# fchchen/omni-recall-rag

Measured on AMD Instinct MI355X. Metric: queries/sec at top-k=10 over N x 3072-d chunks; score delta vs C# reference in `parity`, higher is better.
Workload: dtype i8 screen + f32*f32->f64 exact re-score; 1 GPU; C3: 10000000 chunks x 3072-d fp32 on one GPU, batch=256 queries per step, top-k=10, full hybrid (cosine+keyword+recency), candidate_limit=corpus; corpus_rows=10000000

## Files before the change

omni-recall-rag_amd/csrc/orr_api.hip:

```cpp
#include <hip/hip_runtime.h>

#include <algorithm>
#include <cmath>
#include <cstdarg>
#include <cstdio>
#include <chrono>
#include <pthread.h>
#include <dlfcn.h>
#include <atomic>
#include <condition_variable>
#include <functional>
#include <cstring>
#include <limits>
#include <mutex>
#include <shared_mutex>
#include <deque>
#include <new>
#include <numeric>
#include <string>
#include <string_view>
#include <thread>
#include <unordered_map>
#include <vector>

// ... 95 lines not shown

}

struct orr_index {
    int device = 0;
    int32_t dim = 0;
    int64_t row_base = 0;
    hipStream_t stream = nullptr;
    hipStream_t stream_kw = nullptr;
    hipStream_t stream_aux = nullptr;
    hipEvent_t ev_bm_clean = nullptr;
    bool bm_clean_pending = false;
    bool kw_counters_clean = false;
    const void *kw_counters_of[2] = {nullptr, nullptr};
    hipEvent_t ev_inputs = nullptr, ev_kw_done = nullptr, ev_main_ready = nullptr, ev_range[15] = {};
    std::mutex mu;

    int64_t n_rows = 0, cap_rows = 0;
    float *d_emb = nullptr;
    int64_t *d_created = nullptr;
    int64_t *d_row_ids = nullptr;
    uint64_t *d_cstart = nullptr;
    uint32_t *d_clen = nullptr;
    uint8_t *d_pool = nullptr;
    uint64_t pool_len = 0, pool_cap = 0;
    double *d_norm_b = nullptr;
    int64_t n_tokens = 0;
    uint8_t *d_vpool = nullptr;
    uint64_t *d_vstart = nullptr;
    uint32_t *d_vlen = nullptr;
// ... 22 lines not shown
    int opt_shard_pass = 0;
    int opt_shard_topk = 0;
    int sample_boost = 1;
    DevBuf emb_shadow;
    bool shadow_ready = false, shadow_failed = false;
    DevBuf emb_i8, i8_scale, i8_rel_err, i8_rel_hat, i8_rowf;
    bool i8_ready = false, i8_failed = false;
    std::vector<int64_t> dead;
    DevBuf d_dead;
    int64_t dead_before = 0;
    const orr_index *parent = nullptr;
    std::vector<std::pair<int64_t, int64_t>> id_index;

    DevBuf ws_q, ws_dot, ws_dotf, ws_sel, ws_cand, ws_qc, ws_rowc, ws_tau, ws_qsplit, ws_fcnt, ws_fbuf, ws_fqf, ws_fany, ws_tsL, ws_tskey, ws_qtiled, ws_fdot, ws_pbuf, ws_psel, ws_q8, ws_q8s1, ws_q8err, ws_zero, ws_norm_a;
    DevBuf ws_keys_a, ws_keys_b, ws_vals_a, ws_vals_b, ws_sort_tmp, ws_raw, ws_src_start, ws_qsub;
    DevBuf ws_vmatch, ws_bitmaps, ws_hits, ws_counter, ws_meta, ws_tickets, ws_kwalias;
    size_t bitmaps_clean = 0;
    const void *bitmaps_clean_of = nullptr;
    PinnedBuf pin_meta, pin_q, pin_qc, pin_cand, pin_norm, pin_cnt, pin_kwcnt;
    hipEvent_t ev_q = nullptr;

    LanePool lanes{this};
    bool internal_lane = false;
    std::atomic<int> user_views{0};

    int profiling = 0;
    std::vector<KernelStat> stats;
    std::vector<PendingEvent> pending;
    std::vector<hipEvent_t> event_pool;
};

// ... 342 lines not shown
    HIP_TRY(hipGetDeviceProperties(&prop, cfg->device));
    if (strncmp(prop.gcnArchName, "gfx950", 6) != 0)
        return fail(ORR_EDEVICE, "device %d is %s; this library carries gfx950 code only", cfg->device, prop.gcnArchName);
    orr_index *idx = new (std::nothrow) orr_index();
    if (!idx) return fail(ORR_ENOMEM, "out of host memory");
    idx->device = cfg->device;
    idx->dim = cfg->dim;
    idx->row_base = cfg->row_base;
    if (hipSetDevice(idx->device) != hipSuccess || hipStreamCreateWithFlags(&idx->stream, hipStreamNonBlocking) != hipSuccess ||
        hipStreamCreateWithFlags(&idx->stream_kw, hipStreamNonBlocking) != hipSuccess ||
        hipStreamCreateWithFlags(&idx->stream_aux, hipStreamNonBlocking) != hipSuccess ||
        hipEventCreateWithFlags(&idx->ev_bm_clean, hipEventDisableTiming) != hipSuccess ||
        hipEventCreateWithFlags(&idx->ev_inputs, hipEventDisableTiming) != hipSuccess ||
        hipEventCreateWithFlags(&idx->ev_kw_done, hipEventDisableTiming) != hipSuccess ||
        hipEventCreateWithFlags(&idx->ev_main_ready, hipEventDisableTiming) != hipSuccess ||
        !create_range_events(idx->ev_range) ||
        hipEventCreateWithFlags(&idx->ev_q, hipEventDisableTiming) != hipSuccess) {
        orr_index_destroy(idx);
        return fail(ORR_EDEVICE, "cannot create streams on device %d", cfg->device);
    }
    if (cfg->capacity_rows > 0) {
        int r = ensure_row_capacity(idx, cfg->capacity_rows);
        if (r != ORR_OK) { orr_index_destroy(idx); return r; }
    }
    *out = idx;
    return ORR_OK;
}

void orr_index_destroy(orr_index *idx)
{
// ... 5 lines not shown
            LanePool::Exclusive all(&idx->lanes);
            views = idx->lanes.drain();
            idx->lanes.set_max_lanes(1);
        }
        for (orr_index *l : views) orr_index_destroy(l);
    }
    (void)hipSetDevice(idx->device);
    if (idx->stream) (void)hipStreamSynchronize(idx->stream);
    if (idx->stream_kw) (void)hipStreamSynchronize(idx->stream_kw);
    if (idx->stream_aux) (void)hipStreamSynchronize(idx->stream_aux);
    if (idx->ev_bm_clean) (void)hipEventDestroy(idx->ev_bm_clean);
    if (idx->stream_aux) (void)hipStreamDestroy(idx->stream_aux);
    if (idx->ev_inputs) (void)hipEventDestroy(idx->ev_inputs);
    if (idx->ev_kw_done) (void)hipEventDestroy(idx->ev_kw_done);
    if (idx->ev_main_ready) (void)hipEventDestroy(idx->ev_main_ready);
    for (hipEvent_t e : idx->ev_range) if (e) (void)hipEventDestroy(e);
    if (idx->stream_kw) (void)hipStreamDestroy(idx->stream_kw);
    for (auto &pe : idx->pending) { (void)hipEventDestroy(pe.start); (void)hipEventDestroy(pe.stop); }
    for (auto e : idx->event_pool) (void)hipEventDestroy(e);
    if (!idx->is_view) {
        if (idx->d_emb) (void)hipFree(idx->d_emb);
        if (idx->d_created) (void)hipFree(idx->d_created);
        if (idx->d_row_ids) (void)hipFree(idx->d_row_ids);
        if (idx->d_cstart) (void)hipFree(idx->d_cstart);
        if (idx->d_clen) (void)hipFree(idx->d_clen);
        if (idx->d_pool) (void)hipFree(idx->d_pool);
        if (idx->d_norm_b) (void)hipFree(idx->d_norm_b);
        if (idx->d_vpool) (void)hipFree(idx->d_vpool);
        if (idx->d_vstart) (void)hipFree(idx->d_vstart);
        if (idx->d_vlen) (void)hipFree(idx->d_vlen);
// ... 866 lines not shown
    v->device = parent->device; v->dim = parent->dim; v->row_base = parent->row_base;
    v->n_rows = parent->n_rows; v->cap_rows = parent->cap_rows;
    v->d_emb = parent->d_emb; v->d_created = parent->d_created; v->d_row_ids = parent->d_row_ids; v->d_norm_b = parent->d_norm_b;
    v->n_tokens = parent->n_tokens; v->d_vpool = parent->d_vpool; v->d_vstart = parent->d_vstart; v->d_vlen = parent->d_vlen;
    v->d_post_off = parent->d_post_off; v->d_post_rows = parent->d_post_rows; v->n_postings = parent->n_postings;
    v->sealed = true;
    copy_options(parent, v);
    borrow_shadows(parent, v);
    if (hipStreamCreateWithFlags(&v->stream, hipStreamNonBlocking) != hipSuccess ||
        hipStreamCreateWithFlags(&v->stream_kw, hipStreamNonBlocking) != hipSuccess ||
        hipStreamCreateWithFlags(&v->stream_aux, hipStreamNonBlocking) != hipSuccess ||
        hipEventCreateWithFlags(&v->ev_bm_clean, hipEventDisableTiming) != hipSuccess ||
        hipEventCreateWithFlags(&v->ev_inputs, hipEventDisableTiming) != hipSuccess ||
        hipEventCreateWithFlags(&v->ev_kw_done, hipEventDisableTiming) != hipSuccess ||
        hipEventCreateWithFlags(&v->ev_main_ready, hipEventDisableTiming) != hipSuccess ||
        !create_range_events(v->ev_range) ||
        hipEventCreateWithFlags(&v->ev_q, hipEventDisableTiming) != hipSuccess) {
        v->internal_lane = true;
        orr_index_destroy(v);
        return fail(ORR_EDEVICE, "cannot create streams on device %d", parent->device);
    }
    v->internal_lane = internal;
    if (!internal) parent->user_views.fetch_add(1);
    *out = v;
    return ORR_OK;
}

int orr_index_screen_dots(orr_index *idx, int32_t B, int32_t dim, const float *q, float *out)
{
    if (!idx || !q || !out || B <= 0) return fail(ORR_EINVAL, "orr_index_screen_dots: bad argument");
// ... 185 lines not shown
    void done()
    {
        if (!on || ++calls % 64 != 0) return;
        fprintf(stderr, "[orr host ms/call] query_setup+cos_launch %.3f | keyword_prep+launch %.3f | norms+consts %.3f | select_launches %.3f | "
                        "wait_gpu %.3f | finish %.3f\n", acc[0] / 64, acc[1] / 64, acc[2] / 64, acc[3] / 64, acc[4] / 64, acc[5] / 64);
        for (double &x : acc) x = 0;
    }
};
thread_local HostTiming g_ht;

struct KwSide {
    orr::KwView view{nullptr, 0, nullptr, nullptr, nullptr};
    size_t bm_bytes = 0, bm_clean_before = 0;
    bool overflow_possible = false;
    uint32_t max_hits = 0;
};

int launch_keyword_side(orr_index *idx, const BatchArgs &a, const std::vector<uint32_t> &qoff, KwSide &out)
{
    const int32_t B = a.B;
    const uint32_t t_begin = qoff[0], n_terms_total = qoff[(size_t)B] - qoff[0];
    if (n_terms_total == 0) return ORR_OK;
    {

        std::vector<std::string_view> dterms;
        dterms.reserve(n_terms_total);
        uint32_t table_size = 16;
        while (table_size < 2 * n_terms_total + 2) table_size <<= 1;
        std::vector<uint32_t> table(table_size, 0xFFFFFFFFu);
        std::vector<uint32_t> qmeta((size_t)n_terms_total + (size_t)B + 1);
// ... 99 lines not shown
        size_t bm_clean = idx->bitmaps_clean_of == idx->ws_bitmaps.p ? idx->bitmaps_clean : 0;
        idx->bitmaps_clean = 0;
        idx->bitmaps_clean_of = idx->ws_bitmaps.p;
        out.bm_clean_before = bm_clean;
        ORR_TRY(idx->ws_hits.reserve(sizeof(orr::KwHit) * (size_t)max_hits));
        ORR_TRY(idx->ws_counter.reserve(sizeof(unsigned long long)));
        ORR_TRY(idx->pin_kwcnt.reserve(sizeof(unsigned long long)));
        *idx->pin_kwcnt.as<unsigned long long>() = 0ull;
        hipStream_t k = idx->stream_kw;
        uint8_t *dm = idx->ws_meta.as<uint8_t>();
        HIP_TRY(hipMemcpyAsync(dm, hm, meta_bytes, hipMemcpyHostToDevice, k));
        const bool counters_clean = idx->kw_counters_clean && idx->kw_counters_of[0] == idx->ws_counter.p;
        idx->kw_counters_clean = false;
        if (!counters_clean) HIP_TRY(hipMemsetAsync(idx->ws_counter.p, 0, sizeof(unsigned long long), k));
        bool bitmaps_settled = false;
        auto settle_bitmaps = [&]() -> int {
            if (bitmaps_settled) return ORR_OK;
            bitmaps_settled = true;
            if (idx->bm_clean_pending) {
                HIP_TRY(hipStreamWaitEvent(k, idx->ev_bm_clean, 0));
                idx->bm_clean_pending = false;
            }
            if (bm_clean < out.bm_bytes)
                HIP_TRY(hipMemsetAsync(static_cast<uint8_t *>(idx->ws_bitmaps.p) + bm_clean, 0, out.bm_bytes - bm_clean, k));
            return ORR_OK;
        };
        if (V > 0) {
            const orr::ScanTerm *d_terms = reinterpret_cast<const orr::ScanTerm *>(dm + off_terms);
            {
                Timed t(idx, "vocab_match", 0.0, k);
                if (vocab_lookup) {
                    const uint32_t *lk = reinterpret_cast<const uint32_t *>(dm + off_lk);
                    HIP_TRY(orr::launch_vocab_match_lookup(idx->d_vpool, idx->d_vstart, idx->d_vlen, V,
                                                           reinterpret_cast<const orr::MatchTerm *>(dm + off_match), lk, lk + 8, lk + 8 + TT,
                                                           reinterpret_cast<const uint32_t *>(dm + off_bloom), idx->d_post_off,
                                                           idx->ws_counter.as<unsigned long long>(), idx->ws_hits.as<orr::KwHit>(), max_hits, k));
                } else {
// ... 16 lines not shown
                {
                    Timed t(idx, "vocab_scan", 0.0, k);
                    HIP_TRY(orr::launch_vocab_scan(idx->d_vpool, idx->vlong_start.as<uint64_t>() + n_mid, idx->vlong_len.as<uint32_t>() + n_mid, VS,
                                                   dm + off_pool, d_terms, (int32_t)TT, reinterpret_cast<const uint32_t *>(dm + off_iota),
                                                   idx->ws_vmatch.as<uint16_t>(), k));
                }
                {
                    Timed t(idx, "vocab_hits", 0.0, k);
                    HIP_TRY(orr::launch_vocab_hits(idx->ws_vmatch.as<uint16_t>(), VS, (int32_t)TT, idx->vlong_id.as<uint32_t>() + n_mid, idx->d_post_off,
                                                   idx->ws_counter.as<unsigned long long>(), idx->ws_hits.as<orr::KwHit>(), max_hits, k));
                }
            }
            const uint8_t *skip = nullptr;
            if (idx->n_tok_bm > 0 && idx->tok_bm_words == words) {
                const size_t o_tok = sizeof(uint32_t) * (size_t)TT, o_off = (2 * o_tok + 7) / 8 * 8, o_alias = o_off + sizeof(int64_t) * (size_t)TT;
                ORR_TRY(idx->ws_kwalias.reserve(o_alias + (size_t)TT + 16));
                uint8_t *wa = idx->ws_kwalias.as<uint8_t>();
                if (!(counters_clean && idx->kw_counters_of[1] == idx->ws_kwalias.p))
                    HIP_TRY(hipMemsetAsync(wa, 0, o_tok, k));
                const int64_t delta = (int64_t)(idx->tok_bm.as<uint32_t>() - idx->ws_bitmaps.as<uint32_t>());
                Timed t(idx, "kw_alias", 0.0, k);
                HIP_TRY(orr::launch_kw_alias(idx->ws_hits.as<orr::KwHit>(), idx->ws_counter.as<unsigned long long>(), max_hits, (int32_t)TT,
                                             idx->tok_bm_index.as<int32_t>(), delta, words, reinterpret_cast<uint32_t *>(wa),
                                             reinterpret_cast<uint32_t *>(wa + o_tok), reinterpret_cast<int64_t *>(wa + o_off), wa + o_alias, k));
                out.view.term_word_off = reinterpret_cast<const int64_t *>(wa + o_off);
                skip = wa + o_alias;
            }
            ORR_TRY(settle_bitmaps());
            {
                Timed t(idx, "expand_hits", 0.0, k);
                HIP_TRY(orr::launch_expand_hits(idx->ws_hits.as<orr::KwHit>(), idx->ws_counter.as<unsigned long long>(), max_hits,
                                                idx->d_post_rows, idx->ws_bitmaps.as<uint32_t>(), words, k,
                                                idx->pin_kwcnt.as<unsigned long long>(), skip));
            }
        }
        ORR_TRY(settle_bitmaps());
        HIP_TRY(hipEventRecord(idx->ev_kw_done, k));
        out.view.bitmaps = idx->ws_bitmaps.as<uint32_t>();
        out.view.words_per_term = words;
        out.view.q_term_idx = reinterpret_cast<const uint32_t *>(dm + off_qmeta);
        out.view.q_term_off = out.view.q_term_idx + n_terms_total;
        out.overflow_possible = want_hits > (uint64_t)max_hits;
        out.max_hits = max_hits;
    }
    return ORR_OK;
}

int run_large_k(orr_index *idx, const BatchArgs &a, int32_t kprime, int64_t n, const double *d_dot, const orr::KwView &kw,
                const orr::QueryConst *qc, orr_candidate *d_cand, hipStream_t s)
{
    const int32_t B = a.B;
    ORR_TRY(idx->ws_keys_a.reserve(sizeof(unsigned long long) * (size_t)n));
    ORR_TRY(idx->ws_keys_b.reserve(sizeof(unsigned long long) * (size_t)n));
    ORR_TRY(idx->ws_vals_a.reserve(sizeof(uint32_t) * (size_t)n));
    ORR_TRY(idx->ws_vals_b.reserve(sizeof(uint32_t) * (size_t)n));
    size_t tmp_bytes = 0;
    HIP_TRY(orr::sort_pairs_desc(nullptr, tmp_bytes, idx->ws_keys_a.as<unsigned long long>(),
                                 idx->ws_keys_b.as<unsigned long long>(), idx->ws_vals_a.as<uint32_t>(),
// ... 43 lines not shown
};

enum class Screen { None, I8Ranges, GemvI8, GemvBf16, Bf16Shadow, Bf16x1 };

struct PassPlan {
    PassForm form = PassForm::Exact;
    Screen screen = Screen::None;
    bool use_cos = false;
    bool use_mfma = false;
    bool q_on_device = false;
    bool dev_norms = false;
    bool prefix_i8 = false;
    bool split_queries = false;
    bool batched_score = false;
    bool rowc_inline = false;
    int32_t fused_sample_seg = 0;
    int64_t dotf_rows = 0;
    int n_ranges = 1;
    int64_t range_row[17] = {};
    int32_t count_bits = 0;
    int prefix_floor_form = 0;
    double approx_eps = 0.0;
    double eps1 = 0.0;

    bool two_stage() const {
        return form == PassForm::TwoStageGemm || form == PassForm::TwoStageStream;
    }
    bool stream() const { return form == PassForm::TwoStageStream; }
    double plane_bytes_per_row(int32_t B) const { return (count_bits == 2 ? 8.0 : 16.0) * (double)((B + 31) / 32); }
    bool fused() const { return fused_sample_seg > 0; }
// ... 49 lines not shown
    p.approx_eps = eps_split_bf16(D);
    if (!two_stage) {
        p.form = p.fused_sample_seg > 0 ? PassForm::SplitFused : PassForm::SplitAll;
        return ORR_OK;
    }
    p.form = PassForm::TwoStageGemm;
    if (idx->opt_two_stage == 1 && D % 128 == 0) {
        ORR_TRY(ensure_i8_shadow(idx));
        p.prefix_i8 = idx->i8_ready;
    }
    if (idx->opt_two_stage == 1 && !p.prefix_i8) ORR_TRY(ensure_shadow(idx));
    p.screen = p.prefix_i8 ? Screen::I8Ranges : (idx->opt_two_stage == 1 && idx->shadow_ready) ? Screen::Bf16Shadow : Screen::Bf16x1;
    if (p.prefix_i8) {
        p.split_queries = false;
        p.approx_eps = kEpsI8;
    } else {
        p.eps1 = eps_plain_bf16(D);
    }
    static const char *prefix_env = getenv("ORR_PREFIX_FULL_RANKING");
    p.prefix_floor_form = (prefix_env && atoi(prefix_env) == 1) ? 0
                          : ((int64_t)p.fused_sample_seg * 16 >= 8 * (int64_t)std::max<int32_t>(1, a.topk) && !(prefix_env && atoi(prefix_env) == 2)) ? 2 : 1;
    const bool has_terms = qoff[(size_t)B] > qoff[0];
    if (has_terms && p.prefix_i8 && n >= (int64_t)2000000) {
        p.n_ranges = B > 256 ? 8 : 4;
        constexpr int64_t kRound = 256 * 256;
        for (int r = 1; r < p.n_ranges; ++r) p.range_row[r] = (n * r / p.n_ranges + kRound / 2) / kRound * kRound;
    }
    uint32_t max_terms = 0;
    for (int32_t b = 0; b < B; ++b) max_terms = std::max(max_terms, qoff[(size_t)b + 1] - qoff[(size_t)b]);
    if (has_terms && max_terms <= 3 && p.prefix_i8 && orr::screen_i8_uses_tile16(B, n, D, (n + 63) / 64 * 64) && !getenv("ORR_COUNT_BITS4"))
// ... 6 lines not shown
    ORR_TRY(plan_form(idx, a, kprime, n, qoff, p));
    assert(!p.fused() || !a.no_fuse);
    assert(!p.use_mfma || !a.force_exact);
    assert(!p.two_stage() || p.fused());
    return ORR_OK;
}

struct PassIo {
    const float *d_q = nullptr;
    double *d_dot = nullptr;
    float *d_dotf = nullptr;
    orr::KwView kw{nullptr, 0, nullptr, nullptr, nullptr};
    const double2 *d_rowc = nullptr;
    orr_candidate *d_cand = nullptr;
    bool direct_host = false;
};

int launch_i8_query_image(orr_index *idx, const float *d_q, int32_t B, bool gemm, hipStream_t s)
{
    ORR_TRY(idx->ws_q8.reserve(2 * (size_t)B * idx->dim));
    ORR_TRY(idx->ws_q8s1.reserve(sizeof(float) * (size_t)B));
    if (!gemm) {
        ORR_TRY(idx->ws_q8err.reserve(sizeof(double) * (size_t)B));
        ORR_TRY(idx->ws_fcnt.reserve(sizeof(uint32_t) * 3 * (size_t)B));
        HIP_TRY(orr::launch_i8_queries(d_q, B, idx->dim, idx->ws_q8.p, idx->ws_q8s1.as<float>(), idx->ws_q8err.as<double>(), s, nullptr,
                                       idx->ws_fcnt.as<uint32_t>(), 3 * B));
        return ORR_OK;
    }
    ORR_TRY(idx->ws_q8err.reserve(2 * sizeof(double) * (size_t)B));
    ORR_TRY(idx->ws_qtiled.reserve(orr::i8_tiled_bytes(B, idx->dim)));
// ... 44 lines not shown
    ORR_TRY(idx->ws_dotf.reserve(sizeof(float) * (size_t)B * (size_t)dotf_rows));
    io.d_dotf = idx->ws_dotf.as<float>();
    if (p.prefix_i8) {
        ORR_TRY(launch_i8_query_image(idx, io.d_q, B, true, s));
        const int64_t pre_rows = std::min<int64_t>(dotf_rows, n);
        Timed t(idx, "screen_i8_prefix", 1.0 * (double)pre_rows * idx->dim + 1.0 * (double)B * idx->dim + 4.0 * (double)B * (double)pre_rows);
        HIP_TRY(orr::launch_screen_i8_dots(idx->ws_qtiled.p, B, idx->emb_i8.p, pre_rows, idx->dim, io.d_dotf, dotf_rows, s));
    } else {
        ORR_TRY(split_queries());
        Timed t(idx, "gemm_dot_bf16x3", 4.0 * (double)dotf_rows * idx->dim + 4.0 * (double)B * idx->dim + 4.0 * (double)B * (double)dotf_rows);
        HIP_TRY(orr::launch_gemm_dot_bf16x3(idx->ws_qsplit.p, B, idx->d_emb, 0, dotf_rows, idx->dim, io.d_dotf, dotf_rows, nullptr, 3, s));
    }
    return ORR_OK;
}

int launch_consts(orr_index *idx, const BatchArgs &a, const PassPlan &p, int64_t n, const std::vector<uint32_t> &qoff,
                  bool download_pending, PassIo &io)
{
    const int32_t B = a.B;
    hipStream_t s = idx->stream;
    if (download_pending) HIP_TRY(hipEventSynchronize(idx->ev_q));
    ORR_TRY(idx->pin_qc.reserve(sizeof(orr::QueryConst) * (size_t)B));
    ORR_TRY(idx->ws_qc.reserve(sizeof(orr::QueryConst) * (size_t)B));
    orr::QueryConst *qc = idx->pin_qc.as<orr::QueryConst>();
    if (p.use_cos && !p.dev_norms) {
        if (a.norms_host) memcpy(idx->h_norm_a.data(), a.norms_host, sizeof(double) * (size_t)B);
        else exact_norms(idx->pin_q.as<float>(), B, a.dim, idx->h_norm_a.data());
    }
    for (int32_t b = 0; b < B; ++b) {
        qc[b].use_cos = p.use_cos ? 1 : 0;
// ... 1 lines not shown
        qc[b].n_terms = (int32_t)(qoff[b + 1] - qoff[b]);
        qc[b].inv_n_terms = qc[b].n_terms > 0 ? 1.0 / (double)qc[b].n_terms : 0.0;
        qc[b].inv_sqrt_na = 0.0;
        if (p.batched_score && p.use_cos && !p.dev_norms) {
            if (qc[b].norm_a <= 0.0) qc[b].use_cos = 0;
            else qc[b].inv_sqrt_na = 1.0 / std::sqrt(qc[b].norm_a);
        }
    }
    if (p.dev_norms) {
        HIP_TRY(hipStreamWaitEvent(s, idx->ev_q, 0));
        HIP_TRY(orr::launch_patch_query_norms(idx->ws_qc.as<orr::QueryConst>(), idx->ws_norm_a.as<double>(), B, p.batched_score, s,
                                              idx->pin_norm.as<double>(), qc));
    } else {
        HIP_TRY(hipMemcpyAsync(idx->ws_qc.p, qc, sizeof(orr::QueryConst) * (size_t)B, hipMemcpyHostToDevice, s));
    }
    if (p.batched_score && !p.rowc_inline) {
        ORR_TRY(idx->ws_rowc.reserve(sizeof(double2) * (size_t)n));
        Timed t(idx, "row_consts", 32.0 * (double)n);
        HIP_TRY(orr::launch_row_consts(idx->d_norm_b, idx->d_created, a.now_ticks, n, idx->ws_rowc.as<double2>(), s));
        io.d_rowc = idx->ws_rowc.as<double2>();
    }
    return ORR_OK;
}

int two_stage_tail(orr_index *idx, const BatchArgs &a, int32_t kprime, int64_t n, PassIo &io, const orr::FusedEpilogue &epi,
                   uint32_t kCap, int32_t buf_lists, bool host_records, size_t rec_bytes, hipStream_t s)
{
    const int32_t B = a.B;
    ORR_TRY(idx->ws_fdot.reserve(sizeof(double) * (size_t)B * kCap));
    ORR_TRY(idx->pin_cnt.reserve(sizeof(uint32_t) * (size_t)B));
    if (B <= kFinishFusedMaxB && idx->dim % 256 == 0) {
        if (host_records && !a.out_dev && rec_bytes <= (256u << 10)) {
            ORR_TRY(idx->pin_cand.reserve(rec_bytes));
            io.d_cand = idx->pin_cand.as<orr_candidate>();
            io.direct_host = true;
        }
// ... 24 lines not shown
            HIP_TRY(orr::launch_records_dot_from_buffer(epi.buf, idx->ws_fdot.as<double>(), epi.cnt, kCap, B, kprime, idx->row_base,
                                                        io.d_cand, s));
        }
        HIP_TRY(hipMemcpyAsync(idx->pin_cnt.p, epi.cnt, sizeof(uint32_t) * (size_t)B, hipMemcpyDeviceToHost, s));
    }
    return ORR_OK;
}

int screen_i8_in_ranges(orr_index *idx, const BatchArgs &a, const PassPlan &p, int64_t n, const orr::KwView &kw,
                        orr::FusedEpilogue epi, hipStream_t s)
{
    const int32_t B = a.B;
    const int64_t *range_row = p.range_row;
    if (p.n_ranges > 1) {
        hipStream_t k = idx->stream_kw;
        HIP_TRY(hipEventRecord(idx->ev_main_ready, s));
        HIP_TRY(hipStreamWaitEvent(k, idx->ev_main_ready, 0));
        for (int r = 1; r < p.n_ranges; ++r) {
            {
                Timed t(idx, "count_planes", p.plane_bytes_per_row(B) * (double)(range_row[r + 1] - range_row[r]), k);
                HIP_TRY(orr::launch_query_count_planes(kw, B, n, epi.plane_stride, idx->ws_fany.as<uint32_t>(), k, range_row[r],
                                                       range_row[r + 1], epi.count_bits == 2 ? 2 : 4));
            }
            HIP_TRY(hipEventRecord(idx->ev_range[r - 1], k));
        }
    }
    for (int r = 0; r < p.n_ranges; ++r) {
        if (r > 0) HIP_TRY(hipStreamWaitEvent(s, idx->ev_range[r - 1], 0));
        epi.tickets = idx->ws_tickets.as<uint32_t>() + 8 * r;
        const double rows_r = (double)(range_row[r + 1] - range_row[r]);
        Timed t(idx, "screen_i8_fused", rows_r * ((double)idx->dim + 32.0 + (epi.count_planes ? (epi.count_bits == 2 ? 8.0 : 16.0) * (double)((B + 31) / 32) : 0.0)) +
// ... 39 lines not shown
                HIP_TRY(orr::launch_screen_gemv_i8(idx->ws_q8.p, idx->ws_q8s1.as<float>(), idx->ws_q8err.as<double>(), B, idx->emb_i8.p,
                                                   idx->i8_scale.as<float>(), idx->i8_rel_err.as<float>(), idx->i8_rel_hat.as<float>(),
                                                   idx->d_norm_b, idx->d_created, a.now_ticks, pre_rows, idx->dim, pre, true, s));
            else
                HIP_TRY(orr::launch_screen_gemv_bf16(idx->ws_qsplit.p, B, idx->emb_shadow.p, pre_rows, idx->dim, pre, s));
        }
        {
            Timed t(idx, "select_floor", 0.0);
            const int32_t lists_all = (int32_t)(cap_p / orr::kSelWidth);
            const int32_t lists_p = pre_lists ? (int32_t)((pre_rows + orr::kSelWidth - 1) / orr::kSelWidth) : lists_all;
            if (!pre_lists)
                HIP_TRY(orr::launch_buffer_to_lists(pre.buf, pre.cnt, cap_p, B, 0, lists_all, idx->ws_psel.as<orr::SelEntry>(), s));
            HIP_TRY(orr::launch_select_final_sample(idx->ws_psel.as<orr::SelEntry>(), lists_all, lists_p, B, kth, d_tau, s, floor));
        }
    } else {
        {
            Timed t(idx, "select_floor", 0.0);
            HIP_TRY(orr::launch_select_final_sample(idx->ws_sel.as<orr::SelEntry>(), lists_total, p.fused_sample_seg, B, kth, d_tau, s, floor,
                                                    p.prefix_floor_form == 2 ? 1 : 0));
        }
        const bool gemm_i8 = p.screen == Screen::I8Ranges;
        if (gemm_i8) {
            epi.i8_rowf = idx->i8_rowf.as<float4>();
            epi.i8_qs1 = idx->ws_q8s1.as<float>();
        }
        HIP_TRY(orr::launch_fused_query_consts(idx->ws_qc.as<orr::QueryConst>(), idx->ws_tskey.as<unsigned long long>(), B,
                                               idx->ws_fqf.as<float4>(), s, gemm_i8 ? idx->ws_q8s1.as<float>() : nullptr,
                                               gemm_i8 ? idx->ws_q8err.as<double>() + B : nullptr,
                                               gemm_i8 ? idx->ws_fqf.as<float4>() + B : nullptr,
                                               idx->ws_fcnt.as<uint32_t>(), 3 * B, idx->ws_tickets.as<uint32_t>(), 8 * 16));
// ... 126 lines not shown
                                         io.d_dot, io.d_dotf, n, idx->d_norm_b, idx->d_created, idx->d_row_ids, io.kw,
                                         p.use_mfma ? 0 : 1, p.approx_eps, nullptr, nullptr, 0u, nullptr, io.d_cand, s));
    }
    if (p.use_mfma && !p.two_stage()) {
        Timed t(idx, "rescore_exact", (double)B * kprime * 4.0 * idx->dim);
        HIP_TRY(orr::launch_rescore_exact(idx->d_emb, idx->dim, io.d_q, B, kprime, idx->row_base, io.d_cand, s));
    }
    return ORR_OK;
}

int finish_pass(orr_index *idx, const BatchArgs &a, const PassPlan &p, const KwSide &kws, uint32_t n_terms_total)
{
    const int32_t B = a.B;
    HIP_TRY(hipStreamSynchronize(idx->stream));
    if (kws.bm_bytes) {
        if (kws.bm_bytes >= ((size_t)16 << 20)) {
            HIP_TRY(hipMemsetAsync(idx->ws_bitmaps.p, 0, kws.bm_bytes, idx->stream_aux));
            HIP_TRY(hipEventRecord(idx->ev_bm_clean, idx->stream_aux));
            idx->bm_clean_pending = true;
        } else {
            HIP_TRY(hipMemsetAsync(idx->ws_bitmaps.p, 0, kws.bm_bytes, idx->stream_kw));
        }
        idx->bitmaps_clean = std::max(kws.bm_bytes, kws.bm_clean_before);
    }
    if (n_terms_total > 0 && idx->ws_counter.p) {
        HIP_TRY(hipMemsetAsync(idx->ws_counter.p, 0, sizeof(unsigned long long), idx->stream_kw));
        if (idx->ws_kwalias.p) HIP_TRY(hipMemsetAsync(idx->ws_kwalias.p, 0, idx->ws_kwalias.cap, idx->stream_kw));
        idx->kw_counters_clean = true;
        idx->kw_counters_of[0] = idx->ws_counter.p;
        idx->kw_counters_of[1] = idx->ws_kwalias.p;
    }
    if (p.dev_norms) memcpy(idx->h_norm_a.data(), idx->pin_norm.p, sizeof(double) * (size_t)B);
    if (n_terms_total > 0) {
        idx->sstats.kw_hits_total += (int64_t)(*idx->pin_kwcnt.as<unsigned long long>() >> 32);
        idx->sstats.kw_passes += 1;
    }
// ... 87 lines not shown
        for (auto &c : empty) { memset(&c, 0, sizeof(c)); c.row_id = -1; c.order_key = -1; }
        for (int32_t b = 0; b < B; ++b) {
            orr_candidate &t = empty[(size_t)b * (kprime + 1) + kprime];
            t.approx_score = -std::numeric_limits<double>::infinity();
            t.order_key = 0; t.matches = 0; t.flags = ORR_CAND_TRAILER;
        }
        if (io.direct_host) memcpy(io.d_cand, empty.data(), rec_bytes);
        else HIP_TRY(hipMemcpyAsync(io.d_cand, empty.data(), rec_bytes, hipMemcpyHostToDevice, s));
        HIP_TRY(hipStreamSynchronize(s));
        if (q_download_pending || p.dev_norms) HIP_TRY(hipEventSynchronize(idx->ev_q));
        if (recs_host && io.direct_host) *recs_host = io.d_cand;
        return ORR_OK;
    }

    if (p.screen == Screen::GemvI8) ORR_TRY(launch_i8_query_image(idx, io.d_q, B, false, s));

    KwSide kws;
    ORR_TRY(launch_keyword_side(idx, a, qoff, kws));
    io.kw = kws.view;
    g_ht.mark(1);

    ORR_TRY(launch_numerators(idx, a, p, n, io));
    g_ht.mark(0);

    ORR_TRY(launch_consts(idx, a, p, n, qoff, q_download_pending, io));
    if (n_terms_total > 0) HIP_TRY(hipStreamWaitEvent(s, idx->ev_kw_done, 0));
    g_ht.mark(2);

    ORR_TRY(launch_selection(idx, a, p, kprime, n, io, host_records, rec_bytes));

    if (!owner_of(idx)->dead.empty())
        HIP_TRY(orr::launch_mark_dead_records(io.d_cand, B, kprime, owner_of(idx)->d_dead.as<int64_t>(),
                                              (int32_t)owner_of(idx)->dead.size(), idx->row_base, s));
    if (host_records && !io.direct_host) {
        ORR_TRY(idx->pin_cand.reserve(rec_bytes));
        HIP_TRY(hipMemcpyAsync(idx->pin_cand.p, io.d_cand, rec_bytes, hipMemcpyDeviceToHost, s));
    }
    g_ht.mark(3);
    idx->sstats.pass_mode = p.pass_mode();

// ... 867 lines not shown
```

omni-recall-rag_amd/csrc/orr_kernels.h:

```cpp
#pragma once

#include <hip/hip_runtime.h>
#include <stdint.h>

#include "../../include/omnirecall_hip.h"

#include <atomic>

namespace orr {

inline int current_device_ordinal()
{
    int d = 0;
    if (hipGetDevice(&d) != hipSuccess || d < 0) d = 0;
    return d;
}
template <auto KERNEL>
hipError_t ensure_max_dynamic_lds(int bytes)
{
    static std::atomic<uint64_t> done[4] = {};
    const int dev = current_device_ordinal() & 255;
    if ((done[dev >> 6].load(std::memory_order_acquire) >> (dev & 63)) & 1ull) return hipSuccess;
    const hipError_t e = hipFuncSetAttribute(reinterpret_cast<const void *>(KERNEL), hipFuncAttributeMaxDynamicSharedMemorySize, bytes);
    if (e == hipSuccess) done[dev >> 6].fetch_or(1ull << (dev & 63), std::memory_order_release);
// ... 93 lines not shown
{
    uint32_t h = (key ^ (cls * 0x9E3779B9u)) * 2654435761u;
    h ^= h >> 15;
    return h & (uint32_t)(kVocabBloomBits - 1);
}
hipError_t launch_vocab_match_lookup(const uint8_t *vpool, const uint64_t *vstart, const uint32_t *vlen, int64_t n_tokens,
                                     const MatchTerm *terms, const uint32_t *lk, const uint32_t *keys, const uint32_t *tidx,
                                     const uint32_t *bloom, const uint64_t *post_off, unsigned long long *counter, KwHit *hits,
                                     uint32_t max_hits, hipStream_t s);
hipError_t launch_vocab_match_mid(const uint8_t *vpool, const uint64_t *starts, const uint32_t *lens, const uint32_t *ids, int64_t n_list,
                                  const MatchTerm8 *terms, int32_t n_terms, const uint64_t *post_off, unsigned long long *counter,
                                  KwHit *hits, uint32_t max_hits, hipStream_t s);
hipError_t launch_expand_hits(const KwHit *hits, const unsigned long long *counter, uint32_t max_hits,
                              const uint32_t *post_rows, uint32_t *bitmaps, int64_t words_per_term, hipStream_t s,
                              unsigned long long *counter_host = nullptr, const uint8_t *skip_term = nullptr);
hipError_t launch_kw_alias(const KwHit *hits, const unsigned long long *counter, uint32_t max_hits, int32_t n_terms,
                           const int32_t *tok_bm_index, int64_t bm_store_delta, int64_t words_per_term, uint32_t *term_cnt,
                           uint32_t *term_tok, int64_t *term_word_off, uint8_t *alias, hipStream_t s);

struct QueryConst {
    double norm_a;
    double inv_sqrt_na;
    double inv_n_terms;
    int32_t n_terms;
    int32_t use_cos;
};

hipError_t launch_patch_query_norms(QueryConst *qc, const double *norm_a, int32_t B, bool batched, hipStream_t s,
                                    double *norm_host = nullptr,
                                    const QueryConst *qc_host = nullptr);
// ... 131 lines not shown
```

omni-recall-rag_amd/csrc/orr_kernels.hip:

```cpp
#include "orr_kernels.h"
#include "orr_device.h"

#include <hipcub/hipcub.hpp>

#include <cstdlib>

namespace orr {

__global__ __launch_bounds__(256) void row_consts_kernel(const double *__restrict__ norm_b,
                                                         const int64_t *__restrict__ created, int64_t now_ticks,
                                                         int64_t n_rows, double2 *__restrict__ out)
{
    for (int64_t r = (int64_t)blockIdx.x * blockDim.x + threadIdx.x; r < n_rows; r += (int64_t)gridDim.x * blockDim.x) {
        out[r] = row_consts_of(norm_b[r], created[r], now_ticks);
    }
}

__global__ void patch_query_norms_kernel(QueryConst *__restrict__ qc, const double *__restrict__ norm_a, int32_t B, int32_t batched,
                                         double *__restrict__ norm_host, const QueryConst *__restrict__ qc_host)
{
    const int32_t b = blockIdx.x * blockDim.x + threadIdx.x;
    if (b >= B) return;
    const double na = norm_a[b];
    QueryConst c = qc_host ? qc_host[b] : qc[b];
// ... 711 lines not shown
    if (groups > 65535 || blocks > 0x7FFFFFFF) return hipErrorInvalidValue;
    hipLaunchKernelGGL(vocab_match_short_kernel, dim3((unsigned)blocks, (unsigned)groups), dim3(256), 0, s, vpool, vstart, vlen,
                       n_tokens, terms, n_terms, post_off, counter, hits, max_hits);
    return hipGetLastError();
}

hipError_t launch_expand_hits(const KwHit *hits, const unsigned long long *counter, uint32_t max_hits,
                              const uint32_t *post_rows, uint32_t *bitmaps, int64_t words_per_term, hipStream_t s,
                              unsigned long long *counter_host, const uint8_t *skip_term)
{
    hipLaunchKernelGGL(expand_hits_kernel, dim3(1024), dim3(256), 0, s, hits, counter, max_hits, post_rows, bitmaps,
                       words_per_term, counter_host, skip_term);
    return hipGetLastError();
}

template <bool FAST, int LANEMAX>
__global__ __launch_bounds__(1024) void fuse_select_kernel(const double *__restrict__ dot,
                                                           const float *__restrict__ dotf, int64_t dot_stride,
                                                           const double *__restrict__ norm_b,
                                                           const int64_t *__restrict__ created,
                                                           const double2 *__restrict__ row_consts, KwView kw,
                                                           const QueryConst *__restrict__ qcs,
                                                           int64_t now_ticks, int64_t n_rows, int32_t seg_first,
                                                           int32_t n_seg_total,
                                                           const unsigned long long *__restrict__ tau,
                                                           SelEntry *__restrict__ out_sel, I8Prefix i8)
{
    __shared__ SelEntry lists[16][kSelWidth];
    const int lane = threadIdx.x & 63;
    const int wave = threadIdx.x >> 6;
// ... 463 lines not shown
```

Before: 31290 queries/s.

## Launch i8 screen before keyword side, overlap row consts, clear only non-aliased bitmaps

For the i8 prefix screen path, the numerator/screen kernels are now launched before the keyword-side work, and row constants are computed on the auxiliary stream with an event join. The keyword alias skip flags move into their own buffer so a new kernel clears only the bitmap rows of terms that are not aliased to stored token bitmaps, instead of memsetting the whole bitmap area. The main-ready event for the multi-range path is now recorded at a different point. This aims to overlap keyword work with the screen and cut memset traffic, at the cost of more cross-stream ordering that is harder to get right.

```diff
diff --git a/omni-recall-rag_amd/csrc/orr_api.hip b/omni-recall-rag_amd/csrc/orr_api.hip
--- a/omni-recall-rag_amd/csrc/orr_api.hip
+++ b/omni-recall-rag_amd/csrc/orr_api.hip
@@ -133,6 +133,7 @@
     bool kw_counters_clean = false;
     const void *kw_counters_of[2] = {nullptr, nullptr};
     hipEvent_t ev_inputs = nullptr, ev_kw_done = nullptr, ev_main_ready = nullptr, ev_range[15] = {};
+    hipEvent_t ev_rowc = nullptr;
     std::mutex mu;
 
     int64_t n_rows = 0, cap_rows = 0;
@@ -185,7 +186,7 @@
 
     DevBuf ws_q, ws_dot, ws_dotf, ws_sel, ws_cand, ws_qc, ws_rowc, ws_tau, ws_qsplit, ws_fcnt, ws_fbuf, ws_fqf, ws_fany, ws_tsL, ws_tskey, ws_qtiled, ws_fdot, ws_pbuf, ws_psel, ws_q8, ws_q8s1, ws_q8err, ws_zero, ws_norm_a;
     DevBuf ws_keys_a, ws_keys_b, ws_vals_a, ws_vals_b, ws_sort_tmp, ws_raw, ws_src_start, ws_qsub;
-    DevBuf ws_vmatch, ws_bitmaps, ws_hits, ws_counter, ws_meta, ws_tickets, ws_kwalias;
+    DevBuf ws_vmatch, ws_bitmaps, ws_hits, ws_counter, ws_meta, ws_tickets, ws_kwalias, ws_kwskip;
     size_t bitmaps_clean = 0;
     const void *bitmaps_clean_of = nullptr;
     PinnedBuf pin_meta, pin_q, pin_qc, pin_cand, pin_norm, pin_cnt, pin_kwcnt;
@@ -558,6 +559,7 @@
         hipEventCreateWithFlags(&idx->ev_inputs, hipEventDisableTiming) != hipSuccess ||
         hipEventCreateWithFlags(&idx->ev_kw_done, hipEventDisableTiming) != hipSuccess ||
         hipEventCreateWithFlags(&idx->ev_main_ready, hipEventDisableTiming) != hipSuccess ||
+        hipEventCreateWithFlags(&idx->ev_rowc, hipEventDisableTiming) != hipSuccess ||
         !create_range_events(idx->ev_range) ||
         hipEventCreateWithFlags(&idx->ev_q, hipEventDisableTiming) != hipSuccess) {
         orr_index_destroy(idx);
@@ -593,6 +595,7 @@
     if (idx->ev_inputs) (void)hipEventDestroy(idx->ev_inputs);
     if (idx->ev_kw_done) (void)hipEventDestroy(idx->ev_kw_done);
     if (idx->ev_main_ready) (void)hipEventDestroy(idx->ev_main_ready);
+    if (idx->ev_rowc) (void)hipEventDestroy(idx->ev_rowc);
     for (hipEvent_t e : idx->ev_range) if (e) (void)hipEventDestroy(e);
     if (idx->stream_kw) (void)hipStreamDestroy(idx->stream_kw);
     for (auto &pe : idx->pending) { (void)hipEventDestroy(pe.start); (void)hipEventDestroy(pe.stop); }
@@ -1489,6 +1492,7 @@
         hipEventCreateWithFlags(&v->ev_inputs, hipEventDisableTiming) != hipSuccess ||
         hipEventCreateWithFlags(&v->ev_kw_done, hipEventDisableTiming) != hipSuccess ||
         hipEventCreateWithFlags(&v->ev_main_ready, hipEventDisableTiming) != hipSuccess ||
+        hipEventCreateWithFlags(&v->ev_rowc, hipEventDisableTiming) != hipSuccess ||
         !create_range_events(v->ev_range) ||
         hipEventCreateWithFlags(&v->ev_q, hipEventDisableTiming) != hipSuccess) {
         v->internal_lane = true;
@@ -1704,6 +1708,8 @@
     size_t bm_bytes = 0, bm_clean_before = 0;
     bool overflow_possible = false;
     uint32_t max_hits = 0;
+    const uint8_t *skip = nullptr;
+    uint32_t n_dterms = 0;
 };
 
 int launch_keyword_side(orr_index *idx, const BatchArgs &a, const std::vector<uint32_t> &qoff, KwSide &out)
@@ -1833,13 +1839,17 @@
         idx->kw_counters_clean = false;
         if (!counters_clean) HIP_TRY(hipMemsetAsync(idx->ws_counter.p, 0, sizeof(unsigned long long), k));
         bool bitmaps_settled = false;
-        auto settle_bitmaps = [&]() -> int {
-            if (bitmaps_settled) return ORR_OK;
-            bitmaps_settled = true;
+        auto await_clearing = [&]() -> int {
             if (idx->bm_clean_pending) {
                 HIP_TRY(hipStreamWaitEvent(k, idx->ev_bm_clean, 0));
                 idx->bm_clean_pending = false;
             }
+            return ORR_OK;
+        };
+        auto settle_bitmaps = [&]() -> int {
+            if (bitmaps_settled) return ORR_OK;
+            bitmaps_settled = true;
+            ORR_TRY(await_clearing());
             if (bm_clean < out.bm_bytes)
                 HIP_TRY(hipMemsetAsync(static_cast<uint8_t *>(idx->ws_bitmaps.p) + bm_clean, 0, out.bm_bytes - bm_clean, k));
             return ORR_OK;
@@ -1886,17 +1896,21 @@
             const uint8_t *skip = nullptr;
             if (idx->n_tok_bm > 0 && idx->tok_bm_words == words) {
                 const size_t o_tok = sizeof(uint32_t) * (size_t)TT, o_off = (2 * o_tok + 7) / 8 * 8, o_alias = o_off + sizeof(int64_t) * (size_t)TT;
-                ORR_TRY(idx->ws_kwalias.reserve(o_alias + (size_t)TT + 16));
+                ORR_TRY(idx->ws_kwalias.reserve(o_alias));
+                ORR_TRY(idx->ws_kwskip.reserve((size_t)TT + 16));
                 uint8_t *wa = idx->ws_kwalias.as<uint8_t>();
+                ORR_TRY(await_clearing());
                 if (!(counters_clean && idx->kw_counters_of[1] == idx->ws_kwalias.p))
                     HIP_TRY(hipMemsetAsync(wa, 0, o_tok, k));
                 const int64_t delta = (int64_t)(idx->tok_bm.as<uint32_t>() - idx->ws_bitmaps.as<uint32_t>());
                 Timed t(idx, "kw_alias", 0.0, k);
                 HIP_TRY(orr::launch_kw_alias(idx->ws_hits.as<orr::KwHit>(), idx->ws_counter.as<unsigned long long>(), max_hits, (int32_t)TT,
                                              idx->tok_bm_index.as<int32_t>(), delta, words, reinterpret_cast<uint32_t *>(wa),
-                                             reinterpret_cast<uint32_t *>(wa + o_tok), reinterpret_cast<int64_t *>(wa + o_off), wa + o_alias, k));
+                                             reinterpret_cast<uint32_t *>(wa + o_tok), reinterpret_cast<int64_t *>(wa + o_off),
+                                             idx->ws_kwskip.as<uint8_t>(), k));
                 out.view.term_word_off = reinterpret_cast<const int64_t *>(wa + o_off);
-                skip = wa + o_alias;
+                skip = idx->ws_kwskip.as<uint8_t>();
+                out.skip = skip;
             }
             ORR_TRY(settle_bitmaps());
             {
@@ -1914,6 +1928,7 @@
         out.view.q_term_off = out.view.q_term_idx + n_terms_total;
         out.overflow_possible = want_hits > (uint64_t)max_hits;
         out.max_hits = max_hits;
+        out.n_dterms = TT;
     }
     return ORR_OK;
 }
@@ -1987,6 +2002,7 @@
     bool split_queries = false;
     bool batched_score = false;
     bool rowc_inline = false;
+    bool early_main = false;
     int32_t fused_sample_seg = 0;
     int64_t dotf_rows = 0;
     int n_ranges = 1;
@@ -2066,6 +2082,7 @@
     if (p.prefix_i8) {
         p.split_queries = false;
         p.approx_eps = kEpsI8;
+        p.early_main = true;
     } else {
         p.eps1 = eps_plain_bf16(D);
     }
@@ -2102,6 +2119,7 @@
     const double2 *d_rowc = nullptr;
     orr_candidate *d_cand = nullptr;
     bool direct_host = false;
+    bool rowc_on_aux = false;
 };
 
 int launch_i8_query_image(orr_index *idx, const float *d_q, int32_t B, bool gemm, hipStream_t s)
@@ -2176,6 +2194,15 @@
     return ORR_OK;
 }
 
+int launch_row_consts_on(orr_index *idx, const BatchArgs &a, int64_t n, hipStream_t s, PassIo &io)
+{
+    ORR_TRY(idx->ws_rowc.reserve(sizeof(double2) * (size_t)n));
+    Timed t(idx, "row_consts", 32.0 * (double)n, s);
+    HIP_TRY(orr::launch_row_consts(idx->d_norm_b, idx->d_created, a.now_ticks, n, idx->ws_rowc.as<double2>(), s));
+    io.d_rowc = idx->ws_rowc.as<double2>();
+    return ORR_OK;
+}
+
 int launch_consts(orr_index *idx, const BatchArgs &a, const PassPlan &p, int64_t n, const std::vector<uint32_t> &qoff,
                   bool download_pending, PassIo &io)
 {
@@ -2207,12 +2234,7 @@
     } else {
         HIP_TRY(hipMemcpyAsync(idx->ws_qc.p, qc, sizeof(orr::QueryConst) * (size_t)B, hipMemcpyHostToDevice, s));
     }
-    if (p.batched_score && !p.rowc_inline) {
-        ORR_TRY(idx->ws_rowc.reserve(sizeof(double2) * (size_t)n));
-        Timed t(idx, "row_consts", 32.0 * (double)n);
-        HIP_TRY(orr::launch_row_consts(idx->d_norm_b, idx->d_created, a.now_ticks, n, idx->ws_rowc.as<double2>(), s));
-        io.d_rowc = idx->ws_rowc.as<double2>();
-    }
+    if (p.batched_score && !p.rowc_inline && !io.rowc_on_aux) ORR_TRY(launch_row_consts_on(idx, a, n, s, io));
     return ORR_OK;
 }
 
@@ -2267,7 +2289,6 @@
     const int64_t *range_row = p.range_row;
     if (p.n_ranges > 1) {
         hipStream_t k = idx->stream_kw;
-        HIP_TRY(hipEventRecord(idx->ev_main_ready, s));
         HIP_TRY(hipStreamWaitEvent(k, idx->ev_main_ready, 0));
         for (int r = 1; r < p.n_ranges; ++r) {
             {
@@ -2337,6 +2358,7 @@
             HIP_TRY(orr::launch_select_final_sample(idx->ws_psel.as<orr::SelEntry>(), lists_all, lists_p, B, kth, d_tau, s, floor));
         }
     } else {
+        if (p.screen == Screen::I8Ranges && p.n_ranges > 1) HIP_TRY(hipEventRecord(idx->ev_main_ready, s));
         {
             Timed t(idx, "select_floor", 0.0);
             HIP_TRY(orr::launch_select_final_sample(idx->ws_sel.as<orr::SelEntry>(), lists_total, p.fused_sample_seg, B, kth, d_tau, s, floor,
@@ -2493,12 +2515,15 @@
     const int32_t B = a.B;
     HIP_TRY(hipStreamSynchronize(idx->stream));
     if (kws.bm_bytes) {
-        if (kws.bm_bytes >= ((size_t)16 << 20)) {
-            HIP_TRY(hipMemsetAsync(idx->ws_bitmaps.p, 0, kws.bm_bytes, idx->stream_aux));
+        const bool aux = kws.bm_bytes >= ((size_t)16 << 20);
+        hipStream_t c = aux ? idx->stream_aux : idx->stream_kw;
+        if (kws.skip)
+            HIP_TRY(orr::launch_clear_term_bitmaps(idx->ws_bitmaps.as<uint32_t>(), kws.view.words_per_term, (int32_t)kws.n_dterms, kws.skip, c));
+        else
+            HIP_TRY(hipMemsetAsync(idx->ws_bitmaps.p, 0, kws.bm_bytes, c));
+        if (aux) {
             HIP_TRY(hipEventRecord(idx->ev_bm_clean, idx->stream_aux));
             idx->bm_clean_pending = true;
-        } else {
-            HIP_TRY(hipMemsetAsync(idx->ws_bitmaps.p, 0, kws.bm_bytes, idx->stream_kw));
         }
         idx->bitmaps_clean = std::max(kws.bm_bytes, kws.bm_clean_before);
     }
@@ -2616,16 +2641,26 @@
     }
 
     if (p.screen == Screen::GemvI8) ORR_TRY(launch_i8_query_image(idx, io.d_q, B, false, s));
+    if (p.early_main) {
+        ORR_TRY(launch_numerators(idx, a, p, n, io));
+        if (p.batched_score && !p.rowc_inline) {
+            ORR_TRY(launch_row_consts_on(idx, a, n, idx->stream_aux, io));
+            HIP_TRY(hipEventRecord(idx->ev_rowc, idx->stream_aux));
+            io.rowc_on_aux = true;
+        }
+        g_ht.mark(0);
+    }
 
     KwSide kws;
     ORR_TRY(launch_keyword_side(idx, a, qoff, kws));
     io.kw = kws.view;
     g_ht.mark(1);
 
-    ORR_TRY(launch_numerators(idx, a, p, n, io));
+    if (!p.early_main) ORR_TRY(launch_numerators(idx, a, p, n, io));
     g_ht.mark(0);
 
     ORR_TRY(launch_consts(idx, a, p, n, qoff, q_download_pending, io));
+    if (io.rowc_on_aux) HIP_TRY(hipStreamWaitEvent(s, idx->ev_rowc, 0));
     if (n_terms_total > 0) HIP_TRY(hipStreamWaitEvent(s, idx->ev_kw_done, 0));
     g_ht.mark(2);
 
diff --git a/omni-recall-rag_amd/csrc/orr_kernels.h b/omni-recall-rag_amd/csrc/orr_kernels.h
--- a/omni-recall-rag_amd/csrc/orr_kernels.h
+++ b/omni-recall-rag_amd/csrc/orr_kernels.h
@@ -131,6 +131,7 @@
 hipError_t launch_expand_hits(const KwHit *hits, const unsigned long long *counter, uint32_t max_hits,
                               const uint32_t *post_rows, uint32_t *bitmaps, int64_t words_per_term, hipStream_t s,
                               unsigned long long *counter_host = nullptr, const uint8_t *skip_term = nullptr);
+hipError_t launch_clear_term_bitmaps(uint32_t *bitmaps, int64_t words_per_term, int32_t n_terms, const uint8_t *skip_term, hipStream_t s);
 hipError_t launch_kw_alias(const KwHit *hits, const unsigned long long *counter, uint32_t max_hits, int32_t n_terms,
                            const int32_t *tok_bm_index, int64_t bm_store_delta, int64_t words_per_term, uint32_t *term_cnt,
                            uint32_t *term_tok, int64_t *term_word_off, uint8_t *alias, hipStream_t s);
diff --git a/omni-recall-rag_amd/csrc/orr_kernels.hip b/omni-recall-rag_amd/csrc/orr_kernels.hip
--- a/omni-recall-rag_amd/csrc/orr_kernels.hip
+++ b/omni-recall-rag_amd/csrc/orr_kernels.hip
@@ -749,6 +749,27 @@
     return hipGetLastError();
 }
 
+__global__ __launch_bounds__(256) void clear_term_bitmaps_kernel(uint32_t *__restrict__ bitmaps, int64_t quads_per_term, int32_t n_terms,
+                                                                 const uint8_t *__restrict__ skip_term)
+{
+    for (int32_t t = blockIdx.y; t < n_terms; t += gridDim.y) {
+        if (skip_term[t]) continue;
+        uint4 *bm = reinterpret_cast<uint4 *>(bitmaps) + (int64_t)t * quads_per_term;
+        for (int64_t i = (int64_t)blockIdx.x * blockDim.x + threadIdx.x; i < quads_per_term; i += (int64_t)gridDim.x * blockDim.x)
+            bm[i] = make_uint4(0u, 0u, 0u, 0u);
+    }
+}
+
+hipError_t launch_clear_term_bitmaps(uint32_t *bitmaps, int64_t words_per_term, int32_t n_terms, const uint8_t *skip_term, hipStream_t s)
+{
+    if (n_terms <= 0 || words_per_term <= 0) return hipSuccess;
+    if (!bitmaps || !skip_term || words_per_term % 4 != 0 || (reinterpret_cast<uintptr_t>(bitmaps) & 15u) != 0) return hipErrorInvalidValue;
+    const int64_t quads = words_per_term / 4;
+    const unsigned bx = (unsigned)std::min<int64_t>((quads + 255) / 256, 64), by = (unsigned)std::min<int32_t>(n_terms, 32768);
+    hipLaunchKernelGGL(clear_term_bitmaps_kernel, dim3(bx, by), dim3(256), 0, s, bitmaps, quads, n_terms, skip_term);
+    return hipGetLastError();
+}
+
 template <bool FAST, int LANEMAX>
 __global__ __launch_bounds__(1024) void fuse_select_kernel(const double *__restrict__ dot,
                                                            const float *__restrict__ dotf, int64_t dot_stride,
```

Result: faster. 31630 queries/s, median of 6 (+1.1%).
